# hyeeiin/ECG-Multimodal-Model

Hardware: AMD Instinct MI355X
Metric: samples/sec fwd+bwd, batch-256 multimodal (img+sig+clin), 1->8 MI355X (higher is better)
Workload: dtype bf16; 1 GPU; full multimodal (image 3x224x224 + 5000-pt signal + 16-dim clinical), fwd+bwd+Adam, encoders unfrozen; image_hw=224x224, per_gpu_batch=256, global_batch=256, parallelism=dp1

## Files before the change

### ecg-multimodal-model_amd/csrc/elementwise.hip

```cpp
#include "ops.h"

namespace {

constexpr int EW_THREADS = 256;

__device__ __forceinline__ u32x4 ld16(const void* p) { return *reinterpret_cast<const u32x4*>(p); }
__device__ __forceinline__ u32x4 ld16s(const void* p) {
#ifndef EW_NO_NT
  return __builtin_nontemporal_load(reinterpret_cast<const u32x4*>(p));
#else
  return *reinterpret_cast<const u32x4*>(p);
#endif
}
struct RowDiv { unsigned mul, sh; };
__device__ __forceinline__ long row_div(long r, RowDiv d) { return (long)(((unsigned long long)(unsigned)r * d.mul) >> d.sh); }
static RowDiv make_row_div(int d) {
  unsigned dd = d < 1 ? 1u : (unsigned)d;
  int l = 0;
  while ((1u << l) < dd) ++l;
  RowDiv r;
  r.mul = (unsigned)(((1ull << (31 + l)) + dd - 1) / dd);
  r.sh = 31u + (unsigned)l;
  return r;
}
// ... 213 lines not shown
      const float invstd = (float)(1.0 / sqrt(var + (double)f.eps));
      const float g = f.gamma ? f.gamma[c] : 1.f, b = f.beta ? f.beta[c] : 0.f;
      const float sc = g * invstd;
      const float sh = b - (float)mean * sc;
      s_coef[c - cs.c_lo] = sc;
      s_coef[cs.W + c - cs.c_lo] = sh;
      if (blockIdx.x == 0) {
        f.coef_out[c] = sc;
        f.coef_out[C + c] = sh;
        f.coef_out[2 * C + c] = (float)mean;
        f.coef_out[3 * C + c] = invstd;
        if (f.rm) {
          const double unb = f.count > 1.0 ? var * f.count / (f.count - 1.0) : var;
          f.rm[c] = (1.f - f.momentum) * f.rm[c] + f.momentum * (float)mean;
          f.rv[c] = (1.f - f.momentum) * f.rv[c] + f.momentum * (float)unb;
        }
      }
    }
    __syncthreads();
  }
  if (f.nbt && blockIdx.x == 0 && blockIdx.y == 0 && threadIdx.x == 0) *f.nbt += 1;
}

template <int THREADS>
__device__ __forceinline__ void bn_bwd_fin_prologue(const BnBwdFin& f, const float* __restrict__ coef, int C, ChanSlice cs,
                                                    float* s_bcoef, double* s_red) {
  const int G = C < 128 ? C : 128;
  for (int g0 = cs.c_lo; g0 < cs.c_lo + cs.W; g0 += G) {
    double s1, s2;
    fin_fold_group<THREADS>(f.partial, f.rows, C, g0, G, s_red, s1, s2);
    if ((int)threadIdx.x < G) {
      const int c = g0 + threadIdx.x;
      const float inv = coef[3 * C + c];
      if (f.centered) s2 *= (double)inv;
      s_bcoef[c - cs.c_lo] = (f.gamma ? f.gamma[c] : 1.f) * inv;
      s_bcoef[cs.W + c - cs.c_lo] = (float)(s1 / f.count);
      s_bcoef[2 * cs.W + c - cs.c_lo] = (float)(s2 / f.count);
      if (blockIdx.x == 0) {
        if (f.dgamma) f.dgamma[c] = (float)s2;
        if (f.dbeta) f.dbeta[c] = (float)s1;
      }
    }
    __syncthreads();
  }
}

struct BnActParams {
  const void* y;
  const float* coef;
  const void* res;
  const float* rcoef;
  const float* gate;
  void* out;
  long M;
  int C, rows_per_sample, relu;
  BnFin fin;
  RowDiv rdiv;
  unsigned char* relu_bits;
};

#ifndef BN_ACT_THREADS
#define BN_ACT_THREADS 1024
#endif
template <typename T>
__global__ __launch_bounds__(BN_ACT_THREADS) void bn_act_kernel(BnActParams p) {
  constexpr int VEC = Elem<T>::VEC;
  const ChanSlice cs = chan_slice(p.C);
  const int cpr = cs.W / VEC, rpi = BN_ACT_THREADS / cpr;
  const int chunk = threadIdx.x % cpr, r0 = threadIdx.x / cpr;
  const int c0 = cs.c_lo + chunk * VEC;
  __shared__ double s_red[FIN_LDS_DOUBLES];
  __shared__ float s_coef[2 * 512];
  const float* cf = p.coef + c0;
  int cfs = p.C;
  const T* y = (const T*)p.y;
  const T* res = (const T*)p.res;
  const long stride = (long)gridDim.x * rpi;
  const long rfirst = (long)blockIdx.x * rpi + r0;
  u32x4 py[2] = {}, pr[2] = {};
  bool pre = p.fin.partial != nullptr && rfirst < p.M;
  if (pre) {
    const long q2 = rfirst + stride < p.M ? rfirst + stride : rfirst;
    py[0] = ld16s(y + rfirst * p.C + c0);
    py[1] = ld16s(y + q2 * p.C + c0);
    if (res) {
      pr[0] = ld16s(res + rfirst * p.C + c0);
      pr[1] = ld16s(res + q2 * p.C + c0);
    }
  }
  if (p.fin.partial) {
    bn_fin_prologue<BN_ACT_THREADS>(p.fin, p.C, cs, s_coef, s_red);
    cf = s_coef + chunk * VEC;
    cfs = cs.W;
  }
  float sc[VEC], sh[VEC], rs[VEC], rb[VEC];
#pragma unroll
  for (int j = 0; j < VEC; ++j) {
    sc[j] = cf[j];
    sh[j] = cf[cfs + j];
    rs[j] = p.rcoef ? p.rcoef[c0 + j] : 1.f;
    rb[j] = p.rcoef ? p.rcoef[p.C + c0 + j] : 0.f;
  }
  T* out = (T*)p.out;
  for (long r = rfirst; r < p.M; r += 2 * stride) {
    const long r2 = r + stride;
    const bool two = r2 < p.M;
    const long rb2 = two ? r2 : r;
    u32x4 vy[2], vr[2];
    if (pre) {
      vy[0] = py[0]; vy[1] = py[1]; vr[0] = pr[0]; vr[1] = pr[1];
      pre = false;
    } else {
      vy[0] = ld16s(y + r * p.C + c0);
      vy[1] = ld16s(y + rb2 * p.C + c0);
      if (res) {
        vr[0] = ld16s(res + r * p.C + c0);
        vr[1] = ld16s(res + rb2 * p.C + c0);
      }
    }
#pragma unroll
    for (int u = 0; u < 2; ++u) {
      const long rr = u ? rb2 : r;
      float f[VEC], g[VEC];
      unpack16<T>(vy[u], f);
#pragma unroll
      for (int j = 0; j < VEC; ++j) f[j] = f[j] * sc[j] + sh[j];
      if (p.gate) {
        const float* gp = p.gate + row_div(rr, p.rdiv) * p.C + c0;
#pragma unroll
        for (int j = 0; j < VEC; ++j) f[j] *= gp[j];
      }
      if (res) {
        unpack16<T>(vr[u], g);
#pragma unroll
        for (int j = 0; j < VEC; ++j) f[j] += g[j] * rs[j] + rb[j];
      }
      if (p.relu) {
#pragma unroll
        for (int j = 0; j < VEC; ++j) f[j] = fmaxf(f[j], 0.f);
      }
      if (VEC == 8 && p.relu_bits && (u == 0 || two)) {
        float g[VEC];
        unpack16<T>(pack16<T>(f), g);
        unsigned bits = 0u;
#pragma unroll
        for (int j = 0; j < VEC; ++j) bits |= (g[j] > 0.f ? 1u : 0u) << j;
        p.relu_bits[rr * (p.C / VEC) + c0 / VEC] = (unsigned char)bits;
      }
      if (u == 0 || two) st16(out + rr * p.C + c0, pack16<T>(f));
    }
  }
}

struct BnBwdParams {
  const void* dout;
  const void* maskref;
  const float* gate;
  const float* addc;
  const void* y;
  const float* coef;
  const float* bcoef;
  void* dy;
  void* dz_out;
  float* partial;
  long M;
  int C, rows_per_sample;
  BnBwdFin fin;
  RowDiv rdiv;
  const unsigned char* mask_bits;
};

constexpr int BWD_THREADS = 1024;
template <typename T, bool APPLY>
__global__ __launch_bounds__(BWD_THREADS) void bn_bwd_kernel(BnBwdParams p) {
  constexpr int VEC = Elem<T>::VEC;
  extern __shared__ float shm_dyn[];
  float(*shm)[2 * VEC + 1] = reinterpret_cast<float(*)[2 * VEC + 1]>(shm_dyn);
  const ChanSlice cs = chan_slice(p.C);
  const int cpr = cs.W / VEC, rpi = BWD_THREADS / cpr;
  const int chunk = threadIdx.x % cpr, r0 = threadIdx.x / cpr;
  const int c0 = cs.c_lo + chunk * VEC;
  __shared__ double s_red[APPLY ? FIN_LDS_DOUBLES : 1];
  __shared__ float s_bcoef[APPLY ? 3 * 512 : 1];
  const float* bc = p.bcoef + c0;
  int bcs = p.C;
  const long rfirst = (long)blockIdx.x * rpi + r0;
  u32x4 pd = {}, pv = {};
  bool pre = APPLY && p.fin.partial != nullptr && rfirst < p.M;
  if (pre) {
    pd = ld16s((const T*)p.dout + rfirst * p.C + c0);
    pv = ld16s((const T*)p.y + rfirst * p.C + c0);
  }
  if (APPLY && p.fin.partial) {
    bn_bwd_fin_prologue<BWD_THREADS>(p.fin, p.coef, p.C, cs, s_bcoef, s_red);
    bc = s_bcoef + chunk * VEC;
    bcs = cs.W;
  }
  float mean[VEC], inv[VEC], k1[VEC], k2[VEC], k3[VEC], a1[VEC], a2[VEC], msc[VEC], msh[VEC];
#pragma unroll
  for (int j = 0; j < VEC; ++j) {
    msc[j] = p.coef[c0 + j];
    msh[j] = p.coef[p.C + c0 + j];
    mean[j] = p.coef[2 * p.C + c0 + j];
    inv[j] = p.coef[3 * p.C + c0 + j];
    a1[j] = a2[j] = 0.f;
    if (APPLY) {
      k1[j] = bc[j];
      k2[j] = bc[bcs + j];
      k3[j] = bc[2 * bcs + j];
    }
  }
  const T* dout = (const T*)p.dout;
  const T* mref = (const T*)p.maskref;
  const T* y = (const T*)p.y;
  for (long r = rfirst; r < p.M; r += (long)gridDim.x * rpi) {
    float d[VEC], m[VEC], v[VEC];
    if (pre) {
      unpack16<T>(pd, d);
      unpack16<T>(pv, v);
      pre = false;
    } else {
      unpack16<T>(ld16s(dout + r * p.C + c0), d);
      unpack16<T>(ld16s(y + r * p.C + c0), v);
    }
    if (mref == y) {
#pragma unroll
      for (int j = 0; j < VEC; ++j) d[j] = (v[j] * msc[j] + msh[j]) > 0.f ? d[j] : 0.f;
    } else if (VEC == 8 && p.mask_bits) {
      const unsigned bits = p.mask_bits[r * (p.C / VEC) + c0 / VEC];
#pragma unroll
      for (int j = 0; j < VEC; ++j) d[j] = (bits >> j) & 1u ? d[j] : 0.f;
    } else if (mref) {
      unpack16<T>(ld16s(mref + r * p.C + c0), m);
#pragma unroll
      for (int j = 0; j < VEC; ++j) d[j] = m[j] > 0.f ? d[j] : 0.f;
    }
    if (p.dz_out) st16((T*)p.dz_out + r * p.C + c0, pack16<T>(d));
    if (p.gate) {
      const float* gp = p.gate + row_div(r, p.rdiv) * p.C + c0;
#pragma unroll
      for (int j = 0; j < VEC; ++j) d[j] *= gp[j];
    }
    if (p.addc) {
      const float* ap = p.addc + row_div(r, p.rdiv) * p.C + c0;
#pragma unroll
      for (int j = 0; j < VEC; ++j) d[j] += ap[j];
    }
    if (!APPLY) {
#pragma unroll
      for (int j = 0; j < VEC; ++j) {
        float xh = (v[j] - mean[j]) * inv[j];
        a1[j] += d[j];
        a2[j] += d[j] * xh;
      }
    } else {
      float o[VEC];
#pragma unroll
      for (int j = 0; j < VEC; ++j) {
        float xh = (v[j] - mean[j]) * inv[j];
        o[j] = k1[j] * (d[j] - k2[j] - xh * k3[j]);
      }
      u32x4 pk = pack16<T>(o);
      st16((T*)p.dy + r * p.C + c0, pk);
      if (p.partial) {
        float back[VEC];
        unpack16<T>(pk, back);
#pragma unroll
        for (int j = 0; j < VEC; ++j) a1[j] += back[j];
      }
    }
  }
  if (!APPLY || p.partial) {
    constexpr int NQ = APPLY ? 1 : 2;
#pragma unroll
    for (int j = 0; j < VEC; ++j) {
      shm[threadIdx.x][j] = a1[j];
      if (!APPLY) shm[threadIdx.x][VEC + j] = a2[j];
    }
    __syncthreads();
    for (int o = threadIdx.x; o < NQ * p.C; o += BWD_THREADS) {
      int which = o / p.C, c = o % p.C;
      int ck = c / VEC, j = c % VEC;
      float s = 0.f;
      for (int k = 0; k < rpi; ++k) s += shm[k * cpr + ck][which * VEC + j];
      p.partial[(size_t)blockIdx.x * NQ * p.C + o] = s;
    }
  }
}

__global__ __launch_bounds__(1024) void bn_bwd_finalize_kernel(const float* __restrict__ partial, int rows, int C,
                                                               double count, const float* __restrict__ gamma,
                                                               const float* __restrict__ coef, float* dgamma,
                                                               float* dbeta, float* __restrict__ bcoef, int centered) {
  __shared__ double sh[2][16][64];
  const int c = blockIdx.x * 64 + (threadIdx.x & 63);
  const int slice = threadIdx.x >> 6;
  double s1 = 0.0, s2 = 0.0;
  if (c < C) {
    int r = slice;
    for (; r + 48 < rows; r += 64) {
      float a[4], b[4];
#pragma unroll
      for (int u = 0; u < 4; ++u) {
        const float* row = partial + (size_t)(r + 16 * u) * 2 * C;
        a[u] = row[c];
        b[u] = row[C + c];
      }
#pragma unroll
      for (int u = 0; u < 4; ++u) {
        s1 += (double)a[u];
        s2 += (double)b[u];
      }
    }
    for (; r < rows; r += 16) {
      const float* row = partial + (size_t)r * 2 * C;
      s1 += (double)row[c];
      s2 += (double)row[C + c];
    }
  }
  sh[0][slice][threadIdx.x & 63] = s1;
  sh[1][slice][threadIdx.x & 63] = s2;
  __syncthreads();
  if (slice == 0 && c < C) {
    for (int k = 1; k < 16; ++k) {
      s1 += sh[0][k][threadIdx.x];
      s2 += sh[1][k][threadIdx.x];
    }
    if (centered) s2 *= (double)coef[3 * C + c];
    if (dgamma) dgamma[c] = (float)s2;
    if (dbeta) dbeta[c] = (float)s1;
    bcoef[c] = (gamma ? gamma[c] : 1.f) * coef[3 * C + c];
    bcoef[C + c] = (float)(s1 / count);
    bcoef[2 * C + c] = (float)(s2 / count);
  }
}

__global__ __launch_bounds__(1024) void rows_sum_kernel(const float* __restrict__ partial, int rows, int C, float* out,
                                                        int accumulate) {
  __shared__ double sh[16][64];
  const int c = blockIdx.x * 64 + (threadIdx.x & 63);
  const int slice = threadIdx.x >> 6;
  double s = 0.0;
  if (c < C) {
    int r = slice;
    for (; r + 48 < rows; r += 64) {
      float a[4];
#pragma unroll
      for (int u = 0; u < 4; ++u) a[u] = partial[(size_t)(r + 16 * u) * C + c];
#pragma unroll
      for (int u = 0; u < 4; ++u) s += (double)a[u];
    }
    for (; r < rows; r += 16) s += (double)partial[(size_t)r * C + c];
  }
  sh[slice][threadIdx.x & 63] = s;
  __syncthreads();
  if (slice == 0 && c < C) {
    for (int k = 1; k < 16; ++k) s += sh[k][threadIdx.x];
    out[c] = accumulate ? out[c] + (float)s : (float)s;
  }
}

template <typename T>
__global__ __launch_bounds__(EW_THREADS) void bnrelu_maxpool_kernel(const T* __restrict__ y,
                                                                    const float* __restrict__ coef, T* __restrict__ out,
                                                                    unsigned char* __restrict__ idx, int N, int H,
                                                                    int W, int C, int OH, int OW) {
  constexpr int VEC = Elem<T>::VEC;
  const int cpr = C / VEC;
  long total = (long)N * OH * OW * cpr;
  for (long i = (long)blockIdx.x * blockDim.x + threadIdx.x; i < total; i += (long)gridDim.x * blockDim.x) {
    int chunk = (int)(i % cpr);
    long pix = i / cpr;
    int ow = (int)(pix % OW);
    long t = pix / OW;
    int oh = (int)(t % OH), n = (int)(t / OH);
    int c0 = chunk * VEC;
    float best[VEC];
    int bi[VEC];
    if constexpr (sizeof(T) == 2) {
      unsigned key[VEC];
      float scv[VEC], shv[VEC];
#pragma unroll
      for (int j = 0; j < VEC; ++j) {
        key[j] = 0u;
        scv[j] = coef[c0 + j];
        shv[j] = coef[C + c0 + j];
      }
#pragma unroll
      for (int kh = 0; kh < 3; ++kh) {
        int h = oh * 2 - 1 + kh;
        if ((unsigned)h >= (unsigned)H) continue;
#pragma unroll
        for (int kw = 0; kw < 3; ++kw) {
          int w = ow * 2 - 1 + kw;
          if ((unsigned)w >= (unsigned)W) continue;
          float f[VEC];
          unpack16<T>(ld16(y + (((size_t)n * H + h) * W + w) * C + c0), f);
#pragma unroll
          for (int j = 0; j < VEC; ++j) f[j] = fmaxf(f[j] * scv[j] + shv[j], 0.f);
          const u32x4 r = pack16<bf16_t>(f);
          const unsigned tcode = 15u - (unsigned)(kh * 3 + kw);
#pragma unroll
          for (int q = 0; q < 4; ++q) {
            key[2 * q] = max(key[2 * q], ((r[q] & 0x7fffu) << 4) | tcode);
            key[2 * q + 1] = max(key[2 * q + 1], (((r[q] >> 16) & 0x7fffu) << 4) | tcode);
          }
        }
      }
#pragma unroll
      for (int j = 0; j < VEC; ++j) {
        best[j] = __uint_as_float((key[j] >> 4) << 16);
        bi[j] = 15 - (int)(key[j] & 15u);
      }
    } else {
#pragma unroll
      for (int j = 0; j < VEC; ++j) {
        best[j] = -INFINITY;
        bi[j] = 0;
      }
#pragma unroll
      for (int kh = 0; kh < 3; ++kh) {
        int h = oh * 2 - 1 + kh;
        if ((unsigned)h >= (unsigned)H) continue;
#pragma unroll
        for (int kw = 0; kw < 3; ++kw) {
          int w = ow * 2 - 1 + kw;
          if ((unsigned)w >= (unsigned)W) continue;
          float f[VEC];
          unpack16<T>(ld16(y + (((size_t)n * H + h) * W + w) * C + c0), f);
#pragma unroll
          for (int j = 0; j < VEC; ++j) {
            float a = fmaxf(f[j] * coef[c0 + j] + coef[C + c0 + j], 0.f);
            if (a > best[j]) {
              best[j] = a;
              bi[j] = kh * 3 + kw;
            }
          }
        }
// ... 443 lines not shown
  __syncthreads();
  if (fwd) {
    for (int i = threadIdx.x; i < nco * RS * PACK_T; i += 256) {
      const int ci = i % PACK_T, ct = i / PACK_T, tap = ct % RS, co = ct / RS;
      if (ci < nci) Elem<T>::st(fwd + ((size_t)(co0 + co) * RS + tap) * Cin + ci0 + ci, tile[co][ci * RS + tap]);
    }
  }
  if (dgr) {
    for (int i = threadIdx.x; i < nci * RS * PACK_T; i += 256) {
      const int co = i % PACK_T, ct = i / PACK_T, tap = ct % RS, ci = ct / RS;
      if (co < nco) Elem<T>::st(dgr + ((size_t)(ci0 + ci) * RS + tap) * Cout + co0 + co, tile[co][ci * RS + tap]);
    }
  }
}

template <typename T, bool TO_NHWC>
__global__ __launch_bounds__(256) void nchw_nhwc_kernel(const void* __restrict__ src_, void* __restrict__ dst_, int C,
                                                        long HW) {
  __shared__ float tile[32][33];
  const int n = blockIdx.z;
  const long p0 = (long)blockIdx.x * 32;
  const int c0 = blockIdx.y * 32;
  const int tx = threadIdx.x & 31, ty = threadIdx.x >> 5;
  if (TO_NHWC) {
    const float* src = (const float*)src_ + (size_t)n * C * HW;
    T* dst = (T*)dst_ + (size_t)n * C * HW;
    for (int k = ty; k < 32; k += 8) {
      int c = c0 + k;
      long pp = p0 + tx;
      tile[k][tx] = (c < C && pp < HW) ? src[(size_t)c * HW + pp] : 0.f;
    }
    __syncthreads();
    for (int k = ty; k < 32; k += 8) {
      long pp = p0 + k;
      int c = c0 + tx;
      if (c < C && pp < HW) Elem<T>::st(dst + (size_t)pp * C + c, tile[tx][k]);
    }
  } else {
    const T* src = (const T*)src_ + (size_t)n * C * HW;
    float* dst = (float*)dst_ + (size_t)n * C * HW;
    for (int k = ty; k < 32; k += 8) {
      long pp = p0 + k;
      int c = c0 + tx;
      tile[k][tx] = (c < C && pp < HW) ? Elem<T>::ld(src + (size_t)pp * C + c) : 0.f;
    }
    __syncthreads();
    for (int k = ty; k < 32; k += 8) {
      int c = c0 + k;
      long pp = p0 + tx;
      if (c < C && pp < HW) dst[(size_t)c * HW + pp] = tile[tx][k];
    }
  }
}

template <typename T>
__global__ void cast_kernel(const float* __restrict__ src, T* __restrict__ dst, long n) {
  for (long i = (long)blockIdx.x * blockDim.x + threadIdx.x; i < n; i += (long)gridDim.x * blockDim.x)
    Elem<T>::st(dst + i, src[i]);
}
template <typename T>
__global__ void uncast_kernel(const T* __restrict__ src, float* __restrict__ dst, long n) {
  for (long i = (long)blockIdx.x * blockDim.x + threadIdx.x; i < n; i += (long)gridDim.x * blockDim.x)
    dst[i] = Elem<T>::ld(src + i);
}

inline int ew_grid(long work_items, int per_block) {
  long b = (work_items + per_block - 1) / per_block;
  if (b > 4096) b = 4096;
  if (b < 1) b = 1;
  return (int)b;
}
inline bool chunk_ok(int C, int dtype) {
  int vec = dtype == ECGMM_BF16 ? 8 : 4;
  if (C % vec) return false;
  int cpr = C / vec;
  return cpr <= EW_THREADS && (EW_THREADS % cpr) == 0;
}

}

#define DISPATCH_T(dtype, CALL_BF16, CALL_F32, what)                 \
  if ((dtype) == ECGMM_BF16) { CALL_BF16; }                          \
  else if ((dtype) == ECGMM_F32) { CALL_F32; }                       \
  else ECG_FAIL(ECGMM_ERR_DTYPE, what ": bad dtype %d", (int)(dtype))

int ecg_bn_rows(int dtype, long M, int C) {
  int vec = dtype == ECGMM_BF16 ? 8 : 4;
  if (C < vec) return 1;
  int rpi = EW_THREADS / (C / vec);
  int g = ew_grid(M, rpi * 8);
  return g > 1024 ? 1024 : g;
}

static int fold_rows(const float*& partial, int& rows, int width, hipStream_t stream) {
  if (rows <= 512) return 0;
  float* tail = const_cast<float*>(partial) + (size_t)rows * width;
  int chunk = ceil_div(rows, ECG_TAIL_ROWS);
  int nb = ceil_div(rows, chunk);
  hipLaunchKernelGGL(rows_stage1_kernel, dim3(ceil_div(width, 64), nb), dim3(1024), 0, stream, partial, rows, width,
                     chunk, tail);
  ECG_CHECK_LAUNCH("rows_stage1");
  partial = tail;
  rows = nb;
  return 0;
}

int ecg_bn_finalize(const float* partial, int rows, int C, double count, const float* gamma, const float* beta,
                    float* rm, float* rv, long long* nbt, float momentum, float eps, float* coef,
                    hipStream_t stream) {
  ECG_TRY(fold_rows(partial, rows, 2 * C, stream));
  hipLaunchKernelGGL(bn_finalize_kernel, dim3(ceil_div(C, 64)), dim3(1024), 0, stream, partial, rows, C, count, gamma,
                     beta, rm, rv, nbt, momentum, eps, coef);
  ECG_CHECK_LAUNCH("bn_finalize");
  return 0;
}

int ecg_bn_eval_coef(int C, const float* gamma, const float* beta, const float* rm, const float* rv, float eps,
                     float* coef, hipStream_t stream) {
  hipLaunchKernelGGL(bn_eval_coef_kernel, dim3(ceil_div(C, 256)), dim3(256), 0, stream, C, gamma, beta, rm, rv, eps,
                     coef);
  ECG_CHECK_LAUNCH("bn_eval_coef");
  return 0;
}

int ecg_col_stats(int dtype, const void* x, long M, int C, float* partial, int* rows_out, hipStream_t stream) {
  if (!chunk_ok(C, dtype)) ECG_FAIL(ECGMM_ERR_SHAPE, "col_stats: C=%d unsupported", C);
  int grid = ecg_bn_rows(dtype, M, C);
  *rows_out = grid;
  DISPATCH_T(dtype,
             hipLaunchKernelGGL(col_stats_kernel<bf16_t>, dim3(grid), dim3(EW_THREADS), 0, stream, (const bf16_t*)x, M,
                                C, partial),
             hipLaunchKernelGGL(col_stats_kernel<float>, dim3(grid), dim3(EW_THREADS), 0, stream, (const float*)x, M, C,
                                partial),
             "col_stats");
  ECG_CHECK_LAUNCH("col_stats");
  return 0;
}

bool ecg_bn_fold_ok(int C, int rows) {
  if (!sw::BN_FOLD.get() || rows < 1 || rows > 512 || C > 512) return false;
  return C >= 128 ? C % 128 == 0 : (C >= 16 && 1024 % C == 0);
}

static int bn_fold_slices(int C) {
  return sw::BN_FOLD_SLICE.get() && C >= 256 && C % 128 == 0 ? C / 128 : 1;
}
static dim3 bn_fold_grid(int dtype, long M, int C, int ns, int threads, int trips) {
  const int vec = dtype == ECGMM_BF16 ? 8 : 4;
  int gx = ew_grid(M, (threads / (C / ns / vec)) * trips);
  if (gx > 256 / ns) gx = 256 / ns;
  return dim3(gx, ns);
}

int ecg_bn_act_fold(int dtype, const void* y, float* coef, const EcgBnFold& f, const void* res, const float* rcoef,
                    const float* gate, int rows_per_sample, int relu, void* out, long M, int C, hipStream_t stream,
                    unsigned char* relu_bits) {
  if (!chunk_ok(C, dtype)) ECG_FAIL(ECGMM_ERR_SHAPE, "bn_act: C=%d unsupported", C);
  if (!ecg_bn_fold_ok(C, f.rows)) ECG_FAIL(ECGMM_ERR_SHAPE, "bn_act_fold: C=%d rows=%d not foldable", C, f.rows);
  BnActParams p;
  memset(&p, 0, sizeof(p));
  p.y = y; p.coef = coef; p.res = res; p.rcoef = rcoef; p.gate = gate; p.out = out; p.M = M; p.C = C;
  p.rows_per_sample = rows_per_sample > 0 ? rows_per_sample : 1; p.relu = relu;
  p.rdiv = make_row_div(p.rows_per_sample);
  p.fin.partial = f.partial; p.fin.rows = f.rows; p.fin.count = f.count; p.fin.gamma = f.gamma; p.fin.beta = f.beta;
  p.fin.rm = f.rm; p.fin.rv = f.rv; p.fin.nbt = f.nbt; p.fin.momentum = f.momentum; p.fin.eps = f.eps; p.fin.coef_out = coef;
  p.relu_bits = dtype == ECGMM_BF16 && relu ? relu_bits : nullptr;
  const dim3 grid = bn_fold_grid(dtype, M, C, bn_fold_slices(C), BN_ACT_THREADS, 4);
  DISPATCH_T(dtype, hipLaunchKernelGGL(bn_act_kernel<bf16_t>, grid, dim3(BN_ACT_THREADS), 0, stream, p),
             hipLaunchKernelGGL(bn_act_kernel<float>, grid, dim3(BN_ACT_THREADS), 0, stream, p), "bn_act");
  ECG_CHECK_LAUNCH("bn_act_fold");
  return 0;
}

int ecg_bn_act(int dtype, const void* y, const float* coef, const void* res, const float* rcoef, const float* gate,
               int rows_per_sample, int relu, void* out, long M, int C, hipStream_t stream, unsigned char* relu_bits) {
  if (!chunk_ok(C, dtype)) ECG_FAIL(ECGMM_ERR_SHAPE, "bn_act: C=%d unsupported", C);
  BnActParams p;
  memset(&p, 0, sizeof(p));
  p.y = y; p.coef = coef; p.res = res; p.rcoef = rcoef; p.gate = gate; p.out = out; p.M = M; p.C = C;
  p.rows_per_sample = rows_per_sample > 0 ? rows_per_sample : 1; p.relu = relu;
  p.rdiv = make_row_div(p.rows_per_sample);
  p.relu_bits = dtype == ECGMM_BF16 && relu ? relu_bits : nullptr;
  int vec = dtype == ECGMM_BF16 ? 8 : 4;
  int grid = ew_grid(M, (BN_ACT_THREADS / (C / vec)) * 4);
  if (grid > 256) grid = 256;
  DISPATCH_T(dtype, hipLaunchKernelGGL(bn_act_kernel<bf16_t>, dim3(grid), dim3(BN_ACT_THREADS), 0, stream, p),
             hipLaunchKernelGGL(bn_act_kernel<float>, dim3(grid), dim3(BN_ACT_THREADS), 0, stream, p), "bn_act");
  ECG_CHECK_LAUNCH("bn_act");
  return 0;
}

static int bn_bwd_rows(int dtype, long M, int C) {
  int vec = dtype == ECGMM_BF16 ? 8 : 4;
  if (C < vec) return 1;
  int rpi = BWD_THREADS / (C / vec);
  int g = ew_grid(M, rpi * 8);
  return g > 256 ? 256 : g;
}
template <typename T, bool APPLY>
static void bn_bwd_launch(const BnBwdParams& p, dim3 grid, hipStream_t stream) {
  constexpr size_t lds = (size_t)BWD_THREADS * (2 * Elem<T>::VEC + 1) * sizeof(float);
  static bool attr_set = false;
  if (!attr_set) {
    (void)hipFuncSetAttribute((const void*)bn_bwd_kernel<T, APPLY>, hipFuncAttributeMaxDynamicSharedMemorySize, (int)lds);
    attr_set = true;
  }
  hipLaunchKernelGGL((bn_bwd_kernel<T, APPLY>), grid, dim3(BWD_THREADS), lds, stream, p);
}
static dim3 bn_bwd_apply_grid(int dtype, const BnBwdParams& p, int rows) {
  if (!p.fin.partial || p.partial) return dim3(rows);
  return bn_fold_grid(dtype, p.M, p.C, bn_fold_slices(p.C), BWD_THREADS, 8);
}

size_t ecg_bn_bwd_scratch(int dtype, long M, int C) {
  return ((size_t)(bn_bwd_rows(dtype, M, C) + ECG_TAIL_ROWS) * 2 * C + 3 * C) * sizeof(float);
}

int ecg_bn_bwd(int dtype, const void* dout, const void* maskref, const float* gate, const float* addc,
               int rows_per_sample, const void* y, const float* coef, const float* gamma, float* dgamma, float* dbeta,
               void* dy, void* dz_out, float* dbias, long M, int C, float* scratch, hipStream_t stream,
               const unsigned char* mask_bits) {
  if (!chunk_ok(C, dtype)) ECG_FAIL(ECGMM_ERR_SHAPE, "bn_bwd: C=%d unsupported", C);
  if (dtype != ECGMM_BF16 || maskref == y) mask_bits = nullptr;
  int grid = bn_bwd_rows(dtype, M, C);
  float* partial = scratch;
  float* bcoef = scratch + (size_t)(grid + ECG_TAIL_ROWS) * 2 * C;
  BnBwdParams p;
  memset(&p, 0, sizeof(p));
  p.dout = dout; p.maskref = maskref; p.gate = gate; p.addc = addc; p.y = y; p.coef = coef; p.M = M; p.C = C;
  p.rows_per_sample = rows_per_sample > 0 ? rows_per_sample : 1;
  p.rdiv = make_row_div(p.rows_per_sample);
  p.partial = partial;
  p.mask_bits = mask_bits;
  const bool dz_early = dy && dz_out && (mask_bits || (maskref && maskref != y)) && dz_out != dout;
  if (dz_early) p.dz_out = dz_out;
  DISPATCH_T(dtype, (bn_bwd_launch<bf16_t, false>(p, grid, stream)), (bn_bwd_launch<float, false>(p, grid, stream)), "bn_bwd");
  ECG_CHECK_LAUNCH("bn_bwd_reduce");
  const bool fold = dy && !dbias && ecg_bn_fold_ok(C, grid);
  if (!fold) {
    const float* pr = partial;
    int rows = grid;
    hipLaunchKernelGGL(bn_bwd_finalize_kernel, dim3(ceil_div(C, 64)), dim3(1024), 0, stream, pr, rows, C, (double)M,
                       gamma, coef, dgamma, dbeta, bcoef, 0);
    ECG_CHECK_LAUNCH("bn_bwd_finalize");
  }
  if (!dy) return 0;
  p.bcoef = bcoef; p.dy = dy; p.dz_out = dz_out;
  if (fold) {
    p.fin.partial = partial; p.fin.rows = grid; p.fin.count = (double)M; p.fin.gamma = gamma; p.fin.dgamma = dgamma;
    p.fin.dbeta = dbeta; p.fin.centered = 0;
  }
  if (dz_early) { p.dout = dz_out; p.maskref = nullptr; p.mask_bits = nullptr; p.dz_out = nullptr; }
  p.partial = dbias ? partial : nullptr;
  const dim3 agrid = bn_bwd_apply_grid(dtype, p, grid);
  DISPATCH_T(dtype, (bn_bwd_launch<bf16_t, true>(p, agrid, stream)), (bn_bwd_launch<float, true>(p, agrid, stream)), "bn_bwd");
  ECG_CHECK_LAUNCH("bn_bwd_apply");
  if (dbias) {
    hipLaunchKernelGGL(rows_sum_kernel, dim3(ceil_div(C, 64)), dim3(1024), 0, stream, partial, grid, C, dbias, 0);
    ECG_CHECK_LAUNCH("rows_sum");
  }
  return 0;
}

int ecg_bn_bwd_tail(int dtype, const void* dout, const void* maskref, const void* y, const float* coef,
                    const float* gamma, float* dgamma, float* dbeta, void* dy, const float* partial, int rows, long M,
                    int C, float* scratch, hipStream_t stream, const float* gate, const float* addc,
                    int rows_per_sample, float* dbias) {
  if (!chunk_ok(C, dtype)) ECG_FAIL(ECGMM_ERR_SHAPE, "bn_bwd: C=%d unsupported", C);
  if (rows < 1 || rows > 512) ECG_FAIL(ECGMM_ERR_SHAPE, "bn_bwd_tail: %d partial rows (1..512)", rows);
  const int grid = bn_bwd_rows(dtype, M, C);
  float* bcoef = scratch + (size_t)(grid + ECG_TAIL_ROWS) * 2 * C;
  const bool fold = ecg_bn_fold_ok(C, rows);
  if (!fold) {
    hipLaunchKernelGGL(bn_bwd_finalize_kernel, dim3(ceil_div(C, 64)), dim3(1024), 0, stream, partial, rows, C, (double)M,
                       gamma, coef, dgamma, dbeta, bcoef, 1);
    ECG_CHECK_LAUNCH("bn_bwd_finalize");
  }
  BnBwdParams p;
  memset(&p, 0, sizeof(p));
  p.dout = dout; p.maskref = maskref; p.y = y; p.coef = coef; p.M = M; p.C = C;
  p.gate = gate; p.addc = addc; p.rows_per_sample = rows_per_sample > 0 ? rows_per_sample : 1;
  p.rdiv = make_row_div(p.rows_per_sample);
  p.bcoef = bcoef; p.dy = dy;
  if (fold) {
    p.fin.partial = partial; p.fin.rows = rows; p.fin.count = (double)M; p.fin.gamma = gamma; p.fin.dgamma = dgamma;
    p.fin.dbeta = dbeta; p.fin.centered = 1;
  }
  p.partial = dbias ? scratch : nullptr;
  const dim3 agrid = bn_bwd_apply_grid(dtype, p, grid);
  DISPATCH_T(dtype, (bn_bwd_launch<bf16_t, true>(p, agrid, stream)), (bn_bwd_launch<float, true>(p, agrid, stream)), "bn_bwd");
  ECG_CHECK_LAUNCH("bn_bwd_apply");
  if (dbias) {
    hipLaunchKernelGGL(rows_sum_kernel, dim3(ceil_div(C, 64)), dim3(1024), 0, stream, (const float*)scratch, grid, C, dbias, 0);
    ECG_CHECK_LAUNCH("rows_sum");
  }
  return 0;
}

template <typename T>
static void pool_bwd_launch(const void* dp, const void* pooled, const unsigned char* idx, const void* y, const float* coef,
                            const float* gamma, float* dgamma, float* dbeta, void* dy, float* dbias, int N, int H, int W,
                            int C, int OH, int OW, float* scratch, int rows, hipStream_t stream) {
  constexpr int VEC = Elem<T>::VEC;
  constexpr size_t lds2 = (size_t)BWD_THREADS * (2 * VEC + 1) * sizeof(float), ldsp = (size_t)POOL_THREADS * (VEC + 1) * sizeof(float);
  static bool attr_set = false;
  if (!attr_set) {
    (void)hipFuncSetAttribute((const void*)pool_bwd_reduce_kernel<T>, hipFuncAttributeMaxDynamicSharedMemorySize, (int)lds2);
    attr_set = true;
  }
  const long MP = (long)N * OH * OW, M = (long)N * H * W;
  float* partial = scratch;
  float* bcoef = scratch + (size_t)(rows + ECG_TAIL_ROWS) * 2 * C;
  const int rpi = BWD_THREADS / (C / VEC);
  int g1 = ew_grid(MP, rpi * 8);
  g1 = g1 > rows ? rows : g1;
  hipLaunchKernelGGL(pool_bwd_reduce_kernel<T>, dim3(g1), dim3(BWD_THREADS), lds2, stream, (const T*)dp, (const T*)pooled,
                     coef, partial, MP, C);
  hipLaunchKernelGGL(bn_bwd_finalize_kernel, dim3(ceil_div(C, 64)), dim3(1024), 0, stream, (const float*)partial, g1, C,
                     (double)M, gamma, coef, dgamma, dbeta, bcoef, 1);
  const long nblk = (long)N * ((H + 1) / 2) * ((W + 1) / 2);
  int g2 = ew_grid(nblk, POOL_THREADS / (C / VEC));
  if (dbias && g2 > rows) g2 = rows;
  hipLaunchKernelGGL(pool_bn_bwd_apply_kernel<T>, dim3(g2), dim3(POOL_THREADS), dbias ? ldsp : 0, stream, (const T*)dp,
                     (const T*)pooled, idx, (const T*)y, coef, (const float*)bcoef, (T*)dy, dbias ? partial : nullptr, N, H, W,
                     C, OH, OW);
  if (dbias) hipLaunchKernelGGL(rows_sum_kernel, dim3(ceil_div(C, 64)), dim3(1024), 0, stream, (const float*)partial, g2, C, dbias, 0);
}

int ecg_pool_bn_bwd_reduce(int dtype, const void* dp, const void* pooled, const float* coef, const float* gamma, float* dgamma,
                           float* dbeta, int N, int H, int W, int C, float* scratch, const float** bcoef_out,
                           hipStream_t stream) {
  if (dtype != ECGMM_BF16) ECG_FAIL(ECGMM_ERR_DTYPE, "pool_bn_bwd_reduce: bf16 only");
  if (!chunk_ok(C, dtype)) ECG_FAIL(ECGMM_ERR_SHAPE, "pool_bn_bwd_reduce: C=%d unsupported", C);
  using T = bf16_t;
  constexpr int VEC = Elem<T>::VEC;
  constexpr size_t lds2 = (size_t)BWD_THREADS * (2 * VEC + 1) * sizeof(float);
  static bool attr_set = false;
  if (!attr_set) {
    (void)hipFuncSetAttribute((const void*)pool_bwd_reduce_kernel<T>, hipFuncAttributeMaxDynamicSharedMemorySize, (int)lds2);
    attr_set = true;
  }
  const int OH = (H - 1) / 2 + 1, OW = (W - 1) / 2 + 1;
  const int rows = bn_bwd_rows(dtype, (long)N * H * W, C);
  const long MP = (long)N * OH * OW, M = (long)N * H * W;
  float* partial = scratch;
  float* bcoef = scratch + (size_t)(rows + ECG_TAIL_ROWS) * 2 * C;
  const int rpi = BWD_THREADS / (C / VEC);
  int g1 = ew_grid(MP, rpi * 8);
  g1 = g1 > rows ? rows : g1;
  hipLaunchKernelGGL(pool_bwd_reduce_kernel<T>, dim3(g1), dim3(BWD_THREADS), lds2, stream, (const T*)dp, (const T*)pooled, coef,
                     partial, MP, C);
  ECG_CHECK_LAUNCH("pool_bwd_reduce");
  hipLaunchKernelGGL(bn_bwd_finalize_kernel, dim3(ceil_div(C, 64)), dim3(1024), 0, stream, (const float*)partial, g1, C,
                     (double)M, gamma, coef, dgamma, dbeta, bcoef, 1);
  ECG_CHECK_LAUNCH("bn_bwd_finalize");
  *bcoef_out = bcoef;
  return 0;
}

bool ecg_stem_fuse_on() { return sw::STEM_FUSE.get() != 0; }
// ... 195 lines not shown
```

Measured before the change: 39840 samples/s.

## Add software-pipelined specialized BN act and BN backward kernels

Adds new BN forward-activation and BN backward kernels, specialised at compile time on residual, activation and mask variants. Each thread keeps D rows of loads in flight in registers and issues the next fetch right after consuming the current row, with sched barriers to hold the order. The dispatch paths route ungated cases to these kernels and keep the old generic kernels as fallback. This aims to hide memory latency in bandwidth-bound elementwise passes, at the cost of more template instantiations and higher register pressure.

```diff
diff --git a/ecg-multimodal-model_amd/csrc/elementwise.hip b/ecg-multimodal-model_amd/csrc/elementwise.hip
--- a/ecg-multimodal-model_amd/csrc/elementwise.hip
+++ b/ecg-multimodal-model_amd/csrc/elementwise.hip
@@ -389,6 +389,102 @@
   }
 }
 
+template <typename T, int RES, int ACT, int D>
+__global__ __launch_bounds__(BN_ACT_THREADS) void bn_act_pipe_kernel(BnActParams p) {
+  constexpr int VEC = Elem<T>::VEC;
+  const ChanSlice cs = chan_slice(p.C);
+  const int cpr = cs.W / VEC, rpi = BN_ACT_THREADS / cpr;
+  const int chunk = threadIdx.x % cpr, r0 = threadIdx.x / cpr;
+  const int c0 = cs.c_lo + chunk * VEC;
+  __shared__ double s_red[FIN_LDS_DOUBLES];
+  __shared__ float s_coef[2 * 512];
+  const float* cf = p.coef + c0;
+  int cfs = p.C;
+  const T* y = (const T*)p.y;
+  const T* res = (const T*)p.res;
+  T* out = (T*)p.out;
+  const long stride = (long)gridDim.x * rpi;
+  const long rfirst = (long)blockIdx.x * rpi + r0;
+  const long rowstep = stride * p.C;
+  const long offlast = (p.M - 1) * p.C + c0;
+  long qf = rfirst, offf = rfirst * p.C + c0;
+  long rc = rfirst, offc = offf;
+  u32x4 sy[D], sr[RES ? D : 1];
+  auto fetch = [&](u32x4& vy, u32x4& vr) {
+    const long o = qf < p.M ? offf : offlast;
+    vy = ld16s(y + o);
+    if (RES) vr = ld16s(res + o);
+    qf += stride;
+    offf += rowstep;
+  };
+  float sc[VEC], sh[VEC], rs[RES == 2 ? VEC : 1], rb[RES == 2 ? VEC : 1];
+  if (!p.fin.partial) {
+#pragma unroll
+    for (int j = 0; j < VEC; ++j) {
+      sc[j] = cf[j];
+      sh[j] = cf[cfs + j];
+    }
+  }
+  if (RES == 2) {
+#pragma unroll
+    for (int j = 0; j < VEC; ++j) {
+      rs[j] = p.rcoef[c0 + j];
+      rb[j] = p.rcoef[p.C + c0 + j];
+    }
+  }
+#pragma unroll
+  for (int u = 0; u < D; ++u) fetch(sy[u], sr[RES ? u : 0]);
+  if (p.fin.partial) {
+    bn_fin_prologue<BN_ACT_THREADS>(p.fin, p.C, cs, s_coef, s_red);
+    cf = s_coef + chunk * VEC;
+    cfs = cs.W;
+#pragma unroll
+    for (int j = 0; j < VEC; ++j) {
+      sc[j] = cf[j];
+      sh[j] = cf[cfs + j];
+    }
+  }
+  auto consume = [&](const u32x4& vy, const u32x4& vr) {
+    float f[VEC], g[VEC];
+    unpack16<T>(vy, f);
+#pragma unroll
+    for (int j = 0; j < VEC; ++j) f[j] = f[j] * sc[j] + sh[j];
+    if (RES) {
+      unpack16<T>(vr, g);
+#pragma unroll
+      for (int j = 0; j < VEC; ++j) f[j] += g[j] * (RES == 2 ? rs[j] : 1.f) + (RES == 2 ? rb[j] : 0.f);
+    }
+    if (ACT) {
+#pragma unroll
+      for (int j = 0; j < VEC; ++j) f[j] = fmaxf(f[j], 0.f);
+    }
+    const u32x4 pk = pack16<T>(f);
+    if (VEC == 8 && ACT == 2) {
+      float h[VEC];
+      unpack16<T>(pk, h);
+      unsigned bits = 0u;
+#pragma unroll
+      for (int j = 0; j < VEC; ++j) bits |= (h[j] > 0.f ? 1u : 0u) << j;
+      p.relu_bits[offc / VEC] = (unsigned char)bits;
+    }
+    st16(out + offc, pk);
+    rc += stride;
+    offc += rowstep;
+  };
+  while (rc + (D - 1) * stride < p.M) {
+#pragma unroll
+    for (int u = 0; u < D; ++u) {
+      consume(sy[u], sr[RES ? u : 0]);
+      fetch(sy[u], sr[RES ? u : 0]);
+      __builtin_amdgcn_sched_barrier(0);
+    }
+  }
+#pragma unroll
+  for (int u = 0; u < D - 1; ++u) {
+    if (rc < p.M) consume(sy[u], sr[RES ? u : 0]);
+  }
+}
+
 struct BnBwdParams {
   const void* dout;
   const void* maskref;
@@ -521,6 +617,144 @@
       float s = 0.f;
       for (int k = 0; k < rpi; ++k) s += shm[k * cpr + ck][which * VEC + j];
       p.partial[(size_t)blockIdx.x * NQ * p.C + o] = s;
+    }
+  }
+}
+
+enum { BN_MASK_NONE = 0, BN_MASK_Y = 1, BN_MASK_BITS = 2, BN_MASK_REF = 3 };
+template <typename T, bool APPLY, int MASK, bool DZ, int D>
+__global__ __launch_bounds__(BWD_THREADS) void bn_bwd_pipe_kernel(BnBwdParams p) {
+  constexpr int VEC = Elem<T>::VEC;
+  extern __shared__ float shm_dyn[];
+  float(*shm)[2 * VEC + 1] = reinterpret_cast<float(*)[2 * VEC + 1]>(shm_dyn);
+  const ChanSlice cs = chan_slice(p.C);
+  const int cpr = cs.W / VEC, rpi = BWD_THREADS / cpr;
+  const int chunk = threadIdx.x % cpr, r0 = threadIdx.x / cpr;
+  const int c0 = cs.c_lo + chunk * VEC;
+  __shared__ double s_red[APPLY ? FIN_LDS_DOUBLES : 1];
+  __shared__ float s_bcoef[APPLY ? 3 * 512 : 1];
+  const float* bc = p.bcoef + c0;
+  int bcs = p.C;
+  const T* dout = (const T*)p.dout;
+  const T* mref = (const T*)p.maskref;
+  const T* y = (const T*)p.y;
+  const long stride = (long)gridDim.x * rpi;
+  const long rfirst = (long)blockIdx.x * rpi + r0;
+  const long rowstep = stride * p.C;
+  const long offlast = (p.M - 1) * p.C + c0;
+  long qf = rfirst, offf = rfirst * p.C + c0;
+  long rc = rfirst, offc = offf;
+  u32x4 sd[D], sv[D], sm[MASK == BN_MASK_REF ? D : 1];
+  unsigned sb[MASK == BN_MASK_BITS ? D : 1];
+  auto fetch = [&](u32x4& vd, u32x4& vv, u32x4& vm, unsigned& bits) {
+    long o = qf < p.M ? offf : offlast;
+    asm volatile("" : "+v"(o));
+    vd = ld16s(dout + o);
+    vv = ld16s(y + o);
+    if (MASK == BN_MASK_REF) vm = ld16s(mref + o);
+    if (MASK == BN_MASK_BITS) bits = p.mask_bits[o / VEC];
+    qf += stride;
+    offf += rowstep;
+  };
+  float mean[VEC], inv[VEC], k1[APPLY ? VEC : 1], k2[APPLY ? VEC : 1], k3[APPLY ? VEC : 1], a1[APPLY ? 1 : VEC],
+      a2[APPLY ? 1 : VEC], msc[MASK == BN_MASK_Y ? VEC : 1], msh[MASK == BN_MASK_Y ? VEC : 1];
+  auto load_consts = [&]() {
+#pragma unroll
+    for (int j = 0; j < VEC; ++j) {
+      if (MASK == BN_MASK_Y) {
+        msc[j] = p.coef[c0 + j];
+        msh[j] = p.coef[p.C + c0 + j];
+      }
+      mean[j] = p.coef[2 * p.C + c0 + j];
+      inv[j] = p.coef[3 * p.C + c0 + j];
+      if (APPLY) {
+        k1[j] = bc[j];
+        k2[j] = bc[bcs + j];
+        k3[j] = bc[2 * bcs + j];
+      }
+    }
+  };
+#pragma unroll
+  for (int j = 0; j < (APPLY ? 1 : VEC); ++j) a1[j] = a2[j] = 0.f;
+  if (APPLY && p.fin.partial) {
+#pragma unroll
+    for (int u = 0; u < D; ++u) fetch(sd[u], sv[u], sm[MASK == BN_MASK_REF ? u : 0], sb[MASK == BN_MASK_BITS ? u : 0]);
+    bn_bwd_fin_prologue<BWD_THREADS>(p.fin, p.coef, p.C, cs, s_bcoef, s_red);
+    bc = s_bcoef + chunk * VEC;
+    bcs = cs.W;
+    load_consts();
+#pragma unroll
+    for (int j = 0; j < VEC; ++j) {
+      asm volatile("" : "+v"(mean[j]), "+v"(inv[j]));
+      if (MASK == BN_MASK_Y) asm volatile("" : "+v"(msc[j]), "+v"(msh[j]));
+    }
+  } else {
+    load_consts();
+#pragma unroll
+    for (int u = 0; u < D; ++u) fetch(sd[u], sv[u], sm[MASK == BN_MASK_REF ? u : 0], sb[MASK == BN_MASK_BITS ? u : 0]);
+  }
+  auto consume = [&](const u32x4& vd, const u32x4& vv, const u32x4& vm, unsigned bits) {
+    float d[VEC], m[VEC], v[VEC];
+    unpack16<T>(vd, d);
+    unpack16<T>(vv, v);
+    if (MASK == BN_MASK_Y) {
+#pragma unroll
+      for (int j = 0; j < VEC; ++j) d[j] = (v[j] * msc[j] + msh[j]) > 0.f ? d[j] : 0.f;
+    } else if (MASK == BN_MASK_BITS) {
+#pragma unroll
+      for (int j = 0; j < VEC; ++j) d[j] = (bits >> j) & 1u ? d[j] : 0.f;
+    } else if (MASK == BN_MASK_REF) {
+      unpack16<T>(vm, m);
+#pragma unroll
+      for (int j = 0; j < VEC; ++j) d[j] = m[j] > 0.f ? d[j] : 0.f;
+    }
+    if (DZ) st16((T*)p.dz_out + offc, pack16<T>(d));
+    if (!APPLY) {
+#pragma unroll
+      for (int j = 0; j < VEC; ++j) {
+        float xh = (v[j] - mean[j]) * inv[j];
+        a1[j] += d[j];
+        a2[j] += d[j] * xh;
+      }
+#pragma unroll
+      for (int j = 0; j < VEC; ++j) asm volatile("" : "+v"(a1[j]), "+v"(a2[j]));
+    } else {
+      float o[VEC];
+#pragma unroll
+      for (int j = 0; j < VEC; ++j) {
+        float xh = (v[j] - mean[j]) * inv[j];
+        o[j] = k1[j] * (d[j] - k2[j] - xh * k3[j]);
+      }
+      st16((T*)p.dy + offc, pack16<T>(o));
+    }
+    rc += stride;
+    offc += rowstep;
+  };
+  while (rc + (D - 1) * stride < p.M) {
+#pragma unroll
+    for (int u = 0; u < D; ++u) {
+      consume(sd[u], sv[u], sm[MASK == BN_MASK_REF ? u : 0], sb[MASK == BN_MASK_BITS ? u : 0]);
+      fetch(sd[u], sv[u], sm[MASK == BN_MASK_REF ? u : 0], sb[MASK == BN_MASK_BITS ? u : 0]);
+      __builtin_amdgcn_sched_barrier(0);
+    }
+  }
+#pragma unroll
+  for (int u = 0; u < D - 1; ++u) {
+    if (rc < p.M) consume(sd[u], sv[u], sm[MASK == BN_MASK_REF ? u : 0], sb[MASK == BN_MASK_BITS ? u : 0]);
+  }
+  if (!APPLY) {
+#pragma unroll
+    for (int j = 0; j < VEC; ++j) {
+      shm[threadIdx.x][j] = a1[j];
+      shm[threadIdx.x][VEC + j] = a2[j];
+    }
+    __syncthreads();
+    for (int o = threadIdx.x; o < 2 * p.C; o += BWD_THREADS) {
+      int which = o / p.C, c = o % p.C;
+      int ck = c / VEC, j = c % VEC;
+      float s = 0.f;
+      for (int k = 0; k < rpi; ++k) s += shm[k * cpr + ck][which * VEC + j];
+      p.partial[(size_t)blockIdx.x * 2 * p.C + o] = s;
     }
   }
 }
@@ -1270,6 +1504,26 @@
   return dim3(gx, ns);
 }
 
+template <typename T, int RES, int ACT>
+static void bn_act_pipe_launch(const BnActParams& p, dim3 grid, hipStream_t stream) {
+  hipLaunchKernelGGL((bn_act_pipe_kernel<T, RES, ACT, RES ? 2 : 4>), grid, dim3(BN_ACT_THREADS), 0, stream, p);
+}
+template <typename T, int RES>
+static void bn_act_pipe_launch(const BnActParams& p, dim3 grid, hipStream_t stream) {
+  if (!p.relu) return bn_act_pipe_launch<T, RES, 0>(p, grid, stream);
+  if constexpr (Elem<T>::VEC == 8) {
+    if (p.relu_bits) return bn_act_pipe_launch<T, RES, 2>(p, grid, stream);
+  }
+  bn_act_pipe_launch<T, RES, 1>(p, grid, stream);
+}
+template <typename T>
+static void bn_act_launch(const BnActParams& p, dim3 grid, hipStream_t stream) {
+  if (p.gate || p.M < 1) hipLaunchKernelGGL(bn_act_kernel<T>, grid, dim3(BN_ACT_THREADS), 0, stream, p);
+  else if (!p.res) bn_act_pipe_launch<T, 0>(p, grid, stream);
+  else if (!p.rcoef) bn_act_pipe_launch<T, 1>(p, grid, stream);
+  else bn_act_pipe_launch<T, 2>(p, grid, stream);
+}
+
 int ecg_bn_act_fold(int dtype, const void* y, float* coef, const EcgBnFold& f, const void* res, const float* rcoef,
                     const float* gate, int rows_per_sample, int relu, void* out, long M, int C, hipStream_t stream,
                     unsigned char* relu_bits) {
@@ -1284,8 +1538,7 @@
   p.fin.rm = f.rm; p.fin.rv = f.rv; p.fin.nbt = f.nbt; p.fin.momentum = f.momentum; p.fin.eps = f.eps; p.fin.coef_out = coef;
   p.relu_bits = dtype == ECGMM_BF16 && relu ? relu_bits : nullptr;
   const dim3 grid = bn_fold_grid(dtype, M, C, bn_fold_slices(C), BN_ACT_THREADS, 4);
-  DISPATCH_T(dtype, hipLaunchKernelGGL(bn_act_kernel<bf16_t>, grid, dim3(BN_ACT_THREADS), 0, stream, p),
-             hipLaunchKernelGGL(bn_act_kernel<float>, grid, dim3(BN_ACT_THREADS), 0, stream, p), "bn_act");
+  DISPATCH_T(dtype, bn_act_launch<bf16_t>(p, grid, stream), bn_act_launch<float>(p, grid, stream), "bn_act");
   ECG_CHECK_LAUNCH("bn_act_fold");
   return 0;
 }
@@ -1302,8 +1555,7 @@
   int vec = dtype == ECGMM_BF16 ? 8 : 4;
   int grid = ew_grid(M, (BN_ACT_THREADS / (C / vec)) * 4);
   if (grid > 256) grid = 256;
-  DISPATCH_T(dtype, hipLaunchKernelGGL(bn_act_kernel<bf16_t>, dim3(grid), dim3(BN_ACT_THREADS), 0, stream, p),
-             hipLaunchKernelGGL(bn_act_kernel<float>, dim3(grid), dim3(BN_ACT_THREADS), 0, stream, p), "bn_act");
+  DISPATCH_T(dtype, bn_act_launch<bf16_t>(p, dim3(grid), stream), bn_act_launch<float>(p, dim3(grid), stream), "bn_act");
   ECG_CHECK_LAUNCH("bn_act");
   return 0;
 }
@@ -1315,15 +1567,46 @@
   int g = ew_grid(M, rpi * 8);
   return g > 256 ? 256 : g;
 }
+constexpr int bn_bwd_depth(bool apply, int mask, bool dz) {
+  return apply ? (mask == BN_MASK_Y && dz ? 2 : 3) : (mask == BN_MASK_REF && dz ? 3 : 4);
+}
+template <typename T, bool APPLY, int MASK, bool DZ>
+static void bn_bwd_pipe_launch(const BnBwdParams& p, dim3 grid, hipStream_t stream) {
+  constexpr int D = bn_bwd_depth(APPLY, MASK, DZ);
+  constexpr size_t lds = APPLY ? 0 : (size_t)BWD_THREADS * (2 * Elem<T>::VEC + 1) * sizeof(float);
+  static bool attr_set = false;
+  if (lds && !attr_set) {
+    (void)hipFuncSetAttribute((const void*)bn_bwd_pipe_kernel<T, APPLY, MASK, DZ, D>, hipFuncAttributeMaxDynamicSharedMemorySize,
+                              (int)lds);
+    attr_set = true;
+  }
+  hipLaunchKernelGGL((bn_bwd_pipe_kernel<T, APPLY, MASK, DZ, D>), grid, dim3(BWD_THREADS), lds, stream, p);
+}
+template <typename T, bool APPLY, int MASK>
+static void bn_bwd_pipe_launch(const BnBwdParams& p, dim3 grid, hipStream_t stream) {
+  if constexpr (APPLY || MASK == BN_MASK_BITS || MASK == BN_MASK_REF) {
+    if (p.dz_out) return bn_bwd_pipe_launch<T, APPLY, MASK, true>(p, grid, stream);
+  }
+  bn_bwd_pipe_launch<T, APPLY, MASK, false>(p, grid, stream);
+}
 template <typename T, bool APPLY>
 static void bn_bwd_launch(const BnBwdParams& p, dim3 grid, hipStream_t stream) {
-  constexpr size_t lds = (size_t)BWD_THREADS * (2 * Elem<T>::VEC + 1) * sizeof(float);
-  static bool attr_set = false;
-  if (!attr_set) {
-    (void)hipFuncSetAttribute((const void*)bn_bwd_kernel<T, APPLY>, hipFuncAttributeMaxDynamicSharedMemorySize, (int)lds);
-    attr_set = true;
-  }
-  hipLaunchKernelGGL((bn_bwd_kernel<T, APPLY>), grid, dim3(BWD_THREADS), lds, stream, p);
+  if (p.gate || p.addc || (APPLY && p.partial) || p.M < 1) {
+    constexpr size_t lds = (size_t)BWD_THREADS * (2 * Elem<T>::VEC + 1) * sizeof(float);
+    static bool attr_set = false;
+    if (!attr_set) {
+      (void)hipFuncSetAttribute((const void*)bn_bwd_kernel<T, APPLY>, hipFuncAttributeMaxDynamicSharedMemorySize, (int)lds);
+      attr_set = true;
+    }
+    hipLaunchKernelGGL((bn_bwd_kernel<T, APPLY>), grid, dim3(BWD_THREADS), lds, stream, p);
+    return;
+  }
+  if (p.maskref && p.maskref == p.y) return bn_bwd_pipe_launch<T, APPLY, BN_MASK_Y>(p, grid, stream);
+  if constexpr (Elem<T>::VEC == 8) {
+    if (p.mask_bits) return bn_bwd_pipe_launch<T, APPLY, BN_MASK_BITS>(p, grid, stream);
+  }
+  if (p.maskref) return bn_bwd_pipe_launch<T, APPLY, BN_MASK_REF>(p, grid, stream);
+  bn_bwd_pipe_launch<T, APPLY, BN_MASK_NONE>(p, grid, stream);
 }
 static dim3 bn_bwd_apply_grid(int dtype, const BnBwdParams& p, int rows) {
   if (!p.fin.partial || p.partial) return dim3(rows);
```

Result: no change. 40100 samples/s, median of 6 (+0.7%).
